# eichenberger/stereo-svo-slam

Measured on AMD Instinct MI355X. Metric: tracked_frames_per_sec, higher is better.
Workload: dtype f32

## Files before the change

include/svo_hip.h:

```cpp
#ifndef SVO_HIP_H
#define SVO_HIP_H

#include <stddef.h>

#include "svo_types.h"

#ifdef __cplusplus
extern "C" {
#endif

enum {
    SVO_OK = 0,
    SVO_ERR_INVALID = -1,
    SVO_ERR_HIP = -2,
    SVO_ERR_NO_DEVICE = -3,
    SVO_ERR_CAPACITY = -4
};

typedef struct svo_handle svo_handle;

const char *svo_last_error(void);
int svo_version(void);

int svo_handle_create(int device, int max_keypoints, svo_handle **out);
// ... 138 lines not shown
enum { SVO_KERNEL_SIA_GN = 0,
       SVO_KERNEL_REPROJ_GN = 1 };
typedef struct svo_launch_shape {
    int32_t kernel;
    int32_t waves;
    int32_t mode;
    int32_t cap;
    int64_t launches;
} svo_launch_shape;
int svo_ctx_get_launch_shapes(svo_ctx *ctx, svo_launch_shape *out, int max, int *n);
int svo_pick_launch_shapes(const svo_camera_settings *cam, int width, int height, int batch, int n_bound,
                           int rec_cap, int exact, svo_launch_shape out[2]);
int svo_pick_sia_lds_bytes(const svo_camera_settings *cam, int width, int height, int batch, int n_bound,
                           int rec_cap, int exact, int64_t *lds_bytes);

int svo_pinv6_check(svo_handle *h, const float *H_dev, int n, float *out_dev, int32_t *sweeps_dev, int impl);
int svo_solve6_check(svo_handle *h, const float *H_dev, const float *b_dev, int n, float *out_dev,
                     int32_t *sweeps_dev, int impl);

#ifdef __cplusplus
}
#endif
#endif
```

stereo-svo-slam_amd/csrc/klt.hip:

```cpp
#include "svo_kernels.hpp"
#include "klt_bounds.hpp"
#include <cstring>
#include <utility>

namespace svo {

constexpr int KLT_MAX_WIN = 35;
static_assert(KLT_MAX_WIN + 1 <= 36, "largest kernel shape");
#ifndef SVO_KLT_MARGIN
#define SVO_KLT_MARGIN 4
#endif
constexpr int KLT_MARGIN = SVO_KLT_MARGIN;
template <int CW>
struct KltGeom {
    static constexpr int DW = CW;
    static constexpr int RS = 44;
    static constexpr int RROWS = CW + 2;
    static constexpr int TJROWS = DW + 2 * KLT_MARGIN + 2;
    static constexpr int TJS = (DW + 2 * KLT_MARGIN + 6) & ~3;
    static constexpr int J2S = (TJS / 2) | 1;
    static constexpr int J2COPY = ((TJROWS * J2S + 31) / 32) * 32 + 16;
    static constexpr int SD = (DW + 1) * DW;
    static constexpr int SJ2 = J2COPY + TJROWS * J2S;
    static constexpr int SI = (RROWS * RS + 3) / 4;
// ... 113 lines not shown

#define M24(a, b) __mul24((a), (b))

__device__ inline int cv_round(float v) { return (int)rintf(v); }
__device__ inline int cv_floor(float v) { return (int)floorf(v); }

struct LkWeights { v2s top, bot; };

enum { KLT_OUTSIDE = 0, KLT_FLAT = 1, KLT_TRACK = 2 };
struct KltTmplHeader { int state; float A11, A12, A22; double cI1, cI2; };
template <int NPAIR>
struct KltTmpl {
    static constexpr int TQ = (3 * NPAIR + 3) / 4;
    static constexpr int BYTES = TQ * 64 * 16 + 64;
};
__device__ inline LkWeights lk_weights(float fa, float fb) {
    const int W_BITS = 14;
    const int iw00 = cv_round((1.f - fa) * (1.f - fb) * (1 << W_BITS));
    const int iw01 = cv_round(fa * (1.f - fb) * (1 << W_BITS));
    const int iw10 = cv_round((1.f - fa) * fb * (1 << W_BITS));
    const int iw11 = (1 << W_BITS) - iw00 - iw01 - iw10;
    return LkWeights{as_v2s(pack16(iw00, iw01)), as_v2s(pack16(iw10, iw11))};
}

template <int LS, int MAXROWS>
__device__ inline void stage_tile(uint8_t* tile, const ImgView& im, int x0, int y0, int nq, int rows) {
    const int tid = threadIdx.x;
    const bool fast = klt_rect_in_image(x0, y0, 4 * nq, rows, im.w, im.h) &&
                      (((reinterpret_cast<uintptr_t>(im.data) | (uintptr_t)im.stride) & 3) == 0);
    if (fast) {
// ... 87 lines not shown
                    const int gy = reflect101(y0 + min(r + u, rows - 1), im.h);
                    v[u] = im.g()[M24(gy, im.stride) + gx];
                }
#pragma unroll
                for (int u = 0; u < 8; u++)
                    if (r + u < rows) {
                        const uint16_t pv = (uint16_t)((int)v[u] << 7);
                        t16[(r + u) * 2 * KLT_J2S + tcol] = pv;
                        if (tcol > 0) t16[2 * KLT_J2COPY + (r + u) * 2 * KLT_J2S + tcol - 1] = pv;
                    }
            }
        }
    }
}

template <int CW>
__device__ __forceinline__ void klt_track_body(const KltArgs* __restrict__ args) {
    constexpr int NG = KLT_THREADS / CW;
    constexpr int ROWS = CW;
    constexpr int RPT = (((ROWS + NG - 1) / NG) + 1) & ~1;
    constexpr int NPAIR = RPT / 2;
    const KltArgs& a = args[blockIdx.y];
    const int n = *G(a.n_ptr);
    const int kp = blockIdx.x;
    if (kp >= n) return;
    const int tid = threadIdx.x;
#ifdef SVO_KLT_PHASES
    unsigned long long t_phase_ = __builtin_amdgcn_s_memtime();
    KLT_COUNT(8, 1);
#endif
    const int win = a.win;
    const int RW = win + 3, DW = win + 1, TJ = DW + 2 * KLT_MARGIN;
    const int lr = tid / CW, lc = tid - lr * CW;
    const bool row_on = lr < NG;
    const int y0 = row_on ? lr * RPT : 0;

    using GEO = KltGeom<CW>;
    constexpr int KLT_DW = GEO::DW, KLT_RS = GEO::RS, KLT_RROWS = GEO::RROWS, KLT_J2S = GEO::J2S, KLT_J2COPY = GEO::J2COPY;
    __shared__ __attribute__((aligned(16))) int s_mem[GEO::LDS_DWORDS];
    int* const s_d = s_mem;
    uint8_t* const s_I = reinterpret_cast<uint8_t*>(s_mem + GEO::SD);
    uint32_t* const s_J2 = reinterpret_cast<uint32_t*>(s_mem);
    __shared__ double s_part[KLT_WAVES][8];

    const int kfid = __builtin_amdgcn_readfirstlane(a.kf_id ? G(a.kf_id)[kp] : 0);
    SVO_GP(const KfDev) kfp = G(a.kfs) + kfid;

    svo_kp2d ref;
    float nx, ny;
    if (a.proj_pose) {
        const CamD camd = make_camd(a.cam.fx, a.cam.fy, a.cam.cx, a.cam.cy, a.cam);
        svo_kp2d q;
        if (a.proj_mats) {
            const PoseMats pm = *G(a.proj_mats);
            q = project_point(pm.Rd, pm.t, camd, G(a.kps3d)[kp]);
        } else {
            float pose[6];
            for (int i = 0; i < 6; i++) pose[i] = G(a.proj_pose)[i];
            PoseMats pm;
            pose_mats(pose, pm);
            q = project_point(pm.Rd, pm.t, camd, G(a.kps3d)[kp]);
        }
        nx = q.x; ny = q.y;
        ref = G(kfp->kps2d)[G(a.kp_index)[kp]];
        if (tid == 0) {
            G(a.proj_out)[kp] = q;
            if (a.ref_out) G(a.ref_out)[kp] = ref;
        }
    } else {
        ref = G(a.prev_pts)[kp];
        const svo_kp2d q = G(a.cur_pts)[kp];
        nx = q.x; ny = q.y;
    }

    const uint8_t* tmpl_base = (a.proj_pose && kfp->tmpl_win == a.win) ? (const uint8_t*)kfp->tmpl : nullptr;
    const int tmpl_cap = kfp->tmpl_cap;
    SVO_GP(uint8_t) tmpl_valid = G(kfp->tmpl_valid);
    const int kpi = a.proj_pose ? __builtin_amdgcn_readfirstlane(G(a.kp_index)[kp]) : 0;
    const int maxLevel = min(kfp->n_lk, a.n_cur) - 1;
    const float halfWin = (win - 1) * 0.5f;
    const int W_BITS = 14;
    const float FLT_SCALE = 1.f / (1 << 20);
    double epsilon = 0.01;
    epsilon *= epsilon;
    int status = 1;
    float err = 0;
    const bool col_on = row_on && lc < win;

    KLT_PHASE(0);
    for (int level = maxLevel; level >= 0; level--) {
        const ImgView J = a.cur[level];
        const float lscale = (float)(1. / (1 << level));
        float prevx = ref.x * lscale, prevy = ref.y * lscale;
        if (level == maxLevel) { nx = nx * lscale; ny = ny * lscale; }
        else { nx = nx * 2.f; ny = ny * 2.f; }
        float nextx = nx, nexty = ny;

        int tIw[NPAIR], tIx[NPAIR], tIy[NPAIR];
        float A11 = 0, A12 = 0, A22 = 0;
        double cI1 = 0, cI2 = 0;
        int lstate = KLT_TRACK;
        LkWeights wt;
        SVO_GP(uint4) rec = nullptr;
        SVO_GP(uint8_t) vflag = nullptr;
        if (tmpl_base && kpi < tmpl_cap) {
            rec = (SVO_GP(uint4))(tmpl_base + ((size_t)kpi * SVO_LK_LEVELS + level) * KltTmpl<NPAIR>::BYTES);
            vflag = tmpl_valid + kpi * SVO_LK_LEVELS + level;
        }
        KLT_PHASE(5);
        const int TW = (TJ + 3 + 3) & ~3;
        int tx0 = 0, ty0 = 0;
        bool have_tile = false, tile_regs = false;
        KltTileRegs<GEO> pre;
        uint4 hq0 = make_uint4(0, 0, 0, 0), hq1 = hq0;
        uint4 tq[KltTmpl<NPAIR>::TQ];
        int flag = 0;
        if (vflag) {
            flag = *vflag;
            SVO_GP(const uint4) hd = rec + KltTmpl<NPAIR>::TQ * 64;
            hq0 = hd[0]; hq1 = hd[1];
#pragma unroll
            for (int q = 0; q < KltTmpl<NPAIR>::TQ; q++) tq[q] = rec[q * 64 + tid];
            const bool look = klt_corner_in_range(nextx - halfWin, nexty - halfWin, win, J.w, J.h);
            const int px = look ? cv_floor(nextx - halfWin) : 0, py = look ? cv_floor(nexty - halfWin) : 0;
            const int qx0 = (px - KLT_MARGIN) & ~3, qy0 = py - KLT_MARGIN;
            if (look && tile_in_image(J, qx0, qy0, TW >> 2, TJ)) {
                tile_j2_load<GEO>(pre, J, qx0, qy0, TW >> 2, TJ);
                tx0 = qx0; ty0 = qy0; tile_regs = true;
            }
        }
        KLT_PHASE_WAIT(6);
        const bool hit = flag != 0;
        if (hit) {
            static_assert(sizeof(KltTmplHeader) == 32, "two 16-byte loads");
            lstate = (int)hq0.x; A11 = __uint_as_float(hq0.y); A12 = __uint_as_float(hq0.z); A22 = __uint_as_float(hq0.w);
            cI1 = __builtin_bit_cast(double, ((unsigned long long)hq1.y << 32) | hq1.x);
            cI2 = __builtin_bit_cast(double, ((unsigned long long)hq1.w << 32) | hq1.z);
            if (lstate == KLT_TRACK) {
                const uint32_t* f = reinterpret_cast<const uint32_t*>(tq);
#pragma unroll
                for (int k = 0; k < NPAIR; k++) { tIw[k] = (int)f[k]; tIx[k] = (int)f[NPAIR + k]; tIy[k] = (int)f[2 * NPAIR + k]; }
            }
        } else {
        tile_regs = false;
        int lc_b = lc, y0_b = y0;
        asm volatile("" : "+v"(lc_b), "+v"(y0_b));
        const ImgView I = kfp->lk[level];
        prevx -= halfWin; prevy -= halfWin;
        if (!klt_corner_in_range(prevx, prevy, win, I.w, I.h)) {
            lstate = KLT_OUTSIDE;
        } else {
        const int iprevx = cv_floor(prevx), iprevy = cv_floor(prevy);
        wt = lk_weights(prevx - iprevx, prevy - iprevy);

        __syncthreads();
        const int ix0 = (iprevx - 1) & ~3;
        const int ox = iprevx - 1 - ix0;
        stage_tile<KLT_RS, KLT_RROWS>(s_I, I, ix0, iprevy - 1, (ox + RW + 3) >> 2, RW);
// ... 178 lines not shown
                break;
            }
            prevDx = dx; prevDy = dy;
        }
        KLT_PHASE(3);

        if (status && level == 0) {
            const float npx = nx - halfWin, npy = ny - halfWin;
            if (!klt_corner_in_range(npx, npy, win, J.w, J.h)) {
                status = 0;
                continue;
            }
            const int inx = cv_floor(npx), iny = cv_floor(npy);
            if (!have_tile || inx < tx0 || iny < ty0 || inx + DW > tx0 + TW || iny + DW > ty0 + TJ)
                load_tile(inx, iny);
            wt = lk_weights(npx - inx, npy - iny);
            int e = 0;
            if (col_on) {
                int jr[RPT + 1];
                load_pairs(inx - tx0, iny - ty0, jr);
#pragma unroll
                for (int k = 0; k < NPAIR; k++) {
                    const v2s diff = row_pair(jr, wt, k) - as_v2s(tIw[k]);
                    if (y0 + 2 * k < win) e += abs((int)diff.x);
                    if (y0 + 2 * k + 1 < win) e += abs((int)diff.y);
                }
            }
            double sE[1];
            {
                const int pe[1] = {e};
// ... 4 lines not shown
        }
    }

    KLT_PHASE(4);
    if (tid == 0) {
        G(a.cur_pts)[kp] = svo_kp2d{nx, ny};
        G(a.status)[kp] = (uint8_t)status;
        G(a.err)[kp] = status ? err : INFINITY;
    }
}

template <int CW>
__global__ void klt_track_kernel(const KltArgs* __restrict__ args);
template <>
__global__ __launch_bounds__(KLT_THREADS) __attribute__((amdgpu_waves_per_eu(4, 4))) void klt_track_kernel<32>(const KltArgs* __restrict__ args) {
    klt_track_body<32>(args);
}
template <>
__global__ __launch_bounds__(KLT_THREADS) __attribute__((amdgpu_waves_per_eu(2, 2))) void klt_track_kernel<36>(const KltArgs* __restrict__ args) {
    klt_track_body<36>(args);
}

#ifdef SVO_KLT_PHASES
}
extern "C" int svo_debug_klt_phases(unsigned long long* out16) {
    static unsigned long long host[1024][16];
    if (hipMemcpyFromSymbol(host, HIP_SYMBOL(svo::g_klt_phases), sizeof(host)) != hipSuccess) return -1;
    for (int i = 0; i < 16; i++) {
        out16[i] = 0;
        for (int s = 0; s < 1024; s++) out16[i] += host[s][i];
    }
    memset(host, 0, sizeof(host));
    return hipMemcpyToSymbol(HIP_SYMBOL(svo::g_klt_phases), host, sizeof(host)) == hipSuccess ? 0 : -1;
}
namespace svo {
#endif

size_t klt_template_bytes(int win) {
    return win + 1 <= 32 ? KltTmpl<8>::BYTES : KltTmpl<18>::BYTES;
}

void launch_klt(const KltArgs* d_args, int batch, int max_n, int win, hipStream_t stream) {
    if (max_n <= 0) return;
    if (win + 1 <= 32)
        hipLaunchKernelGGL(klt_track_kernel<32>, dim3(max_n, batch), dim3(KLT_THREADS), 0, stream, d_args);
    else
        hipLaunchKernelGGL(klt_track_kernel<36>, dim3(max_n, batch), dim3(KLT_THREADS), 0, stream, d_args);
}

}
```

stereo-svo-slam_amd/csrc/svo_device.hpp:

```cpp
#pragma once

#include <hip/hip_runtime.h>
#include <float.h>
#include <stdint.h>

#include "../../include/svo_types.h"
#include "../../include/svo_libm.h"

namespace svo {

#if defined(__HIP_DEVICE_COMPILE__)
#define SVO_GP(T) __attribute__((address_space(1))) T*
#else
#define SVO_GP(T) T*
#endif
template <class T>
__device__ __forceinline__ SVO_GP(T) G(T* p) { return (SVO_GP(T))p; }

struct ImgView {
    const uint8_t* data;
    int w, h, stride;
    __device__ __forceinline__ SVO_GP(const uint8_t) g() const { return (SVO_GP(const uint8_t))data; }
    __device__ __forceinline__ SVO_GP(uint8_t) gw() const { return (SVO_GP(uint8_t))data; }
};

__host__ __device__ inline ImgView make_view(const svo_image& im) {
    return ImgView{im.data, im.width, im.height, im.stride};
}

#define SVO_LDS(T) __attribute__((address_space(3))) T
template <bool LDS, typename T>
__device__ inline T mem_ld(const T* p, int i) {
// ... 755 lines not shown
```

stereo-svo-slam_amd/csrc/svo_group.hip:

```cpp
#include <hip/hip_runtime.h>

#include <algorithm>
#include <chrono>
#include <cmath>
#include <cstddef>
#include <cstdio>
#include <cstdlib>
#include <cstring>
#include <memory>
#include <new>
#include <vector>

#include "svo_group.hpp"
#include "svo_host.hpp"
#include "svo_tracker.hpp"

using namespace svo;

namespace {

struct PoseFilter {
    static constexpr int N = 12;
    float statePre[N], statePost[N];
    float A[N * N], Hm[N * N], Q[N * N], R[N * N];
// ... 114 lines not shown
};

struct Seq {
    KpsDev kps[2];
    int cur = 0;
    int* d_n = nullptr;
    svo_kp2d* tracked = nullptr;
    float* klt_err = nullptr;
    uint8_t* klt_status = nullptr;
    float* disparity = nullptr;
    float* sia_rec = nullptr;
    float* sia_kpws = nullptr;
    PoseMats* sia_mats = nullptr;
    uint8_t* tmpl_base = nullptr;
    uint8_t* tmpl_valid = nullptr;
    KfDev* d_kfs = nullptr;
    std::vector<KfHost> kfs;
    int kfs_retired = 0;
    DetCell* det = nullptr; int* n_det = nullptr;
    DetCell* sel = nullptr; int* sel_level = nullptr; int* sel_cell = nullptr; int* occupied = nullptr;
    uint32_t* color_lcg = nullptr;
    std::vector<std::unique_ptr<ImageSet>> sets;
    std::vector<ImageSet*> free_sets;
    ImageSet* cur_set = nullptr;
    ImageSet* prev_set = nullptr;
    PoseFilter kf;
    int frame_id = -1;
    int run = 0;
    double ts = 0;
    float pose[6] = {0, 0, 0, 0, 0, 0};
// ... 59 lines not shown
    PinnedPtr<RemapImg> remap_img_host;
    bool timing = false;
    bool failed = false;
    int exact_pinv = 1;
    Event ev[10];
    SetLayout set_layout;
    std::vector<uint8_t*> kf_slabs;
    int kf_slab_count = 0;
    size_t device_bytes = 0;
    std::vector<FinishedRun> finished;
    std::vector<uint8_t*> set_slabs;
    int tmpl_kf = 0, tmpl_cap = 0;
    size_t tmpl_block_bytes = 0, tmpl_valid_bytes = 0;
    svo_totals totals;
    std::vector<svo_launch_shape> launch_shapes;
    bool retire_kf_images = true;
    int image_sets = 0;
    double host_ms[8] = {0, 0, 0, 0, 0, 0, 0, 0};
    long host_steps = 0;
};

void GroupDelete::operator()(svo_group* c) const {
    (void)hipSetDevice(c->device);
    if (c->stream) (void)hipStreamSynchronize(c->stream.get());
    if (std::getenv("SVO_HOST_TIMING") && c->host_steps > 0) {
        static const char* names[7] = {"args", "launch", "pose_filter", "wait_frame", "kf_enqueue", "wait_kf", "bookkeeping"};
        std::fprintf(stderr, "[svo host ms/step over %ld steps]", c->host_steps);
        for (int i = 0; i < 7; i++) std::fprintf(stderr, " %s=%.3f", names[i], c->host_ms[i] / c->host_steps);
        std::fprintf(stderr, "\n");
    }
// ... 244 lines not shown
    c->d_inside = reinterpret_cast<int*>(db + res_bytes + n_bytes);
    return SVO_OK;
}

int alloc_sequence(svo_group* c, Seq& q, int s) {
    q.d_n = c->d_n_all + 2 * s;
    int rc = alloc_kps(c, q.kps[0], q.d_n);
    if (!rc) rc = alloc_kps(c, q.kps[1], q.d_n + 1);
    auto alloc = [&](auto** p, size_t count) { if (!rc) rc = dev_alloc(c, p, count); };
    const size_t cap = c->cap, cells = c->max_cells;
    alloc(&q.tracked, cap); alloc(&q.klt_err, cap); alloc(&q.klt_status, cap); alloc(&q.disparity, cap);
    alloc(&q.sia_rec, sia_rec_ws_floats(c->cam, c->rec_cap)); alloc(&q.sia_kpws, (size_t)9 * c->rec_cap);
    alloc(&q.sia_mats, 1); alloc(&q.d_kfs, c->max_kf);
    alloc(&q.det, SVO_MAX_PYRAMID_LEVELS * cells); alloc(&q.n_det, SVO_MAX_PYRAMID_LEVELS);
    alloc(&q.sel, cells); alloc(&q.sel_level, cells); alloc(&q.sel_cell, cells); alloc(&q.occupied, c->merge_cells);
    alloc(&q.color_lcg, 1);
    if (rc) return rc;
    q.kf.init();
    std::memset(&q.stats, 0, sizeof(q.stats));
    for (int i = 0; i < 4; i++)
        if ((rc = new_image_set(c, q))) return rc;
    return SVO_OK;
}

int alloc_template_cache(svo_group* c) {
    const int B = c->B;
    const int cells = (c->width / c->cam.grid_width) * (c->height / c->cam.grid_height);
    c->tmpl_cap = std::min(c->cap, cells + 64);
    c->tmpl_block_bytes = align_up((size_t)c->tmpl_cap * SVO_LK_LEVELS * klt_template_bytes(c->cam.window_size_opt_flow), 256);
    int K = c->tmpl_block_bytes <= ((size_t)8 << 20) ? 8 : 4;
    if (const char* e = std::getenv("SVO_KLT_CACHE_KF")) K = std::max(0, std::min(std::atoi(e), 64));
// ... 17 lines not shown
}

int grp_create(const svo_camera_settings* cam, int width, int height, int n_sequences, int device, Group* out) {
    int rc = check_settings(cam, width, height, n_sequences);
    if (rc) return rc;
    int count = 0;
    if (hipGetDeviceCount(&count) != hipSuccess || count <= 0)
        return svo_set_error(SVO_ERR_NO_DEVICE, "no HIP device visible: libsvo_hip has no CPU fallback");
    if (device < 0 || device >= count) return svo_set_error(SVO_ERR_INVALID, "device %d out of range", device);
    HIP_TRY(hipSetDevice(device));
    Group g(new (std::nothrow) svo_group());
    svo_group* c = g.get();
    if (!c) return svo_set_error(SVO_ERR_INVALID, "out of host memory");
    c->device = device; c->B = n_sequences; c->width = width; c->height = height; c->cam = *cam;
    std::memset(&c->totals, 0, sizeof(c->totals));
    HIP_TRY(make_stream(c->stream));
    size_group(c);
    if ((rc = alloc_blocks(c))) return rc;
    for (Event& e : c->ev) HIP_TRY(make_event(e));
    c->seqs.resize(n_sequences);
    if ((rc = grow_set_slabs(c, 4 * n_sequences))) return rc;
    for (int s = 0; s < n_sequences; s++)
        if ((rc = alloc_sequence(c, c->seqs[s], s))) return rc;
    if ((rc = grow_kf_slabs(c, std::max(2 * n_sequences, 32)))) return rc;
    if ((rc = alloc_template_cache(c))) return rc;
    HIP_TRY(pinned_malloc(c->remap_img_host, sizeof(RemapImg) * 2 * (size_t)n_sequences));
    c->remap_img.h = c->remap_img_host.get();
    if ((rc = dev_alloc(c, &c->remap_img.d, 2 * (size_t)n_sequences))) return rc;
    HIP_TRY(hipDeviceSynchronize());
    *out = std::move(g);
// ... 168 lines not shown
    const KpsDev& k = q.kps[q.cur];
    sa.left = q.cur_set->left[0]; sa.right = q.cur_set->right;
    sa.n_ptr = k.n; sa.kps2d = k.kps2d; sa.disparity = q.disparity;
    sa.win = c->cam.window_size_depth_calculator; sa.search_x = c->cam.search_x;
    sa.search_y = c->cam.search_y; sa.clamp_half = clamp_half;
    sa.first = 0; sa.first_ptr = first_ptr;
}

void pack_tracking_args(svo_group* c, const Step& st) {
    ArgBlocks& a = c->args;
    for (int slot = 0; slot < (int)st.trk.size(); slot++) {
        const int s = st.trk[slot];
        Seq& q = c->seqs[s];
        FrameResult* dr = c->d_res + s;
        for (int i = 0; i < 6; i++) a.guess.h[s][i] = q.pending ? q.kf.statePost[i] : q.kf.statePre[i];
        pack_compact(c, q, slot, 0).min_kf = &dr->min_kf;
        const KpsDev& k = q.kps[q.cur];
        SiaArgs& sa = clear(a.sia.h[slot]);
        for (int l = 0; l < c->cam.max_pyramid_levels; l++) {
            sa.prev[l] = q.prev_set->left[l];
            sa.cur[l] = q.cur_set->left[l];
        }
        sa.cam = c->cam; sa.n_ptr = k.n; sa.kps2d = k.kps2d; sa.kps3d = k.kps3d; sa.flags = k.flags;
        sa.pose_guess = a.guess.d[s]; sa.pose_out = dr->pose_sia; sa.cost_out = &dr->sia_cost;
        sa.trace = dr->sia_trace; sa.kp_ws = q.sia_kpws;
        sa.rec_ws = q.sia_rec; sa.rec_cap = c->rec_cap;
        sa.mats_out = q.sia_mats;
        sa.dbg_H = nullptr; sa.dbg_level = -1; sa.cap = c->cap; sa.exact_pinv = c->exact_pinv;
        KltArgs& ka = clear(a.klt.h[slot]);
        ka.kfs = q.d_kfs; ka.kf_id = k.kf_id; ka.n_cur = c->n_lk;
        for (int l = 0; l < c->n_lk; l++) ka.cur[l] = q.cur_set->lk[l];
        ka.n_ptr = k.n; ka.prev_pts = nullptr; ka.cur_pts = q.tracked; ka.status = q.klt_status;
        ka.err = q.klt_err; ka.win = c->cam.window_size_opt_flow;
        ka.proj_pose = dr->pose_sia; ka.proj_mats = q.sia_mats; ka.kps3d = k.kps3d; ka.proj_out = k.kps2d;
        ka.kp_index = k.kp_index; ka.ref_out = nullptr; ka.cam = c->cam;
        ReprojArgs& ra = clear(a.reproj.h[slot]);
        ra.cam = c->cam; ra.n_ptr = k.n; ra.kps2d = k.kps2d; ra.kps3d = k.kps3d; ra.flags = k.flags;
        ra.tracked = q.tracked; ra.err = q.klt_err; ra.pose_in = dr->pose_sia;
        ra.pose_out = dr->pose_refined; ra.cost_out = &dr->reproj_cost; ra.trace = &dr->reproj_trace;
        ra.exact_pinv = c->exact_pinv;
        ra.zero_out = c->d_inside + s;
        pack_ssd(c, q, slot, 1, nullptr);
        FilterArgs& fa = clear(a.filter.h[slot]);
        fa.cam = c->cam; fa.n_ptr = k.n; fa.frame_pose = dr->pose_refined;
        fa.kps2d = k.kps2d; fa.kps3d = k.kps3d; fa.flags = k.flags;
        fa.outlier_count = k.outl; fa.inlier_count = k.inl; fa.kf_inv_depth = k.kfx;
        fa.kf_variance = k.kfP; fa.disparity = q.disparity;
        fa.kfs = q.d_kfs; fa.kf_id = k.kf_id; fa.kp_index = k.kp_index;
        fa.do_outlier_check = 1; fa.do_update = 1; fa.do_flags = 1; fa.do_reproject = 1;
        fa.width = c->width; fa.height = c->height; fa.inside_count = c->d_inside + s;
// ... 32 lines not shown
    }
    launch_compact(a.compact.d, T, c->cap, st);
    HIP_TRY(hipGetLastError());
    HIP_TRY(mark(c, 2));
    int grid_n = 1;
    for (int seq : s.trk) grid_n = std::max(grid_n, c->seqs[seq].n_host);
    grid_n = std::min(grid_n, c->cap);
    const LaunchStatus sia_launch =
        launch_sia(a.sia.d, T, c->cam, c->width, c->height, grid_n, c->rec_cap, c->exact_pinv, st);
    HIP_TRY(sia_launch.err);
    if (!sia_launch.shape.fits)
        return svo_set_error(SVO_ERR_CAPACITY, "sparse alignment: %d keypoints exceed the workspaces", grid_n);
    count_launch(c, SVO_KERNEL_SIA_GN, sia_launch.shape);
    HIP_TRY(hipGetLastError());
    HIP_TRY(mark(c, 3));
    launch_klt(a.klt.d, T, grid_n, c->cam.window_size_opt_flow, st);
    HIP_TRY(hipGetLastError());
    HIP_TRY(mark(c, 4));
    const LaunchStatus reproj_launch = launch_reproj(a.reproj.d, T, grid_n, st);
    HIP_TRY(reproj_launch.err);
    if (!reproj_launch.shape.fits)
        return svo_set_error(SVO_ERR_CAPACITY, "reprojection GN: %d keypoints do not fit LDS", grid_n);
    count_launch(c, SVO_KERNEL_REPROJ_GN, reproj_launch.shape);
    HIP_TRY(hipGetLastError());
    HIP_TRY(mark(c, 5));
    launch_ssd(a.ssd.d, T, grid_n, c->cam.window_size_depth_calculator, c->cam.search_y, st);
    HIP_TRY(hipGetLastError());
    HIP_TRY(mark(c, 6));
    launch_filter(a.filter.d, T, grid_n, st);
    HIP_TRY(hipGetLastError());
    HIP_TRY(mark(c, 7));
    HIP_TRY(hipMemcpyAsync(c->h_inside, c->d_inside, sizeof(int) * c->B, hipMemcpyDeviceToHost, st));
// ... 43 lines not shown
    for (int seq = 0; seq < c->B; seq++) {
        if (!s.need[seq]) continue;
        const int rc = pack_keyframe_args(c, m++, seq, s.start[seq] != 0);
        if (rc) return rc;
    }
    if (m == 0) return SVO_OK;
    HIP_TRY(hipMemcpyAsync(a.dev, a.host.get(), a.bytes, hipMemcpyHostToDevice, st));
    launch_compact(a.compact.d, m, c->cap, st);
    HIP_TRY(hipGetLastError());
    if (c->det_levels > 0) {
        launch_detect(a.detect.d, m, c->max_cells, c->det_levels, c->cam.grid_width, c->cam.grid_height, st);
        HIP_TRY(hipGetLastError());
    }
    launch_select_merge(a.merge.d, m, c->max_cells, st);
    HIP_TRY(hipGetLastError());
    launch_ssd(a.ssd.d, m, c->cap, c->cam.window_size_depth_calculator, c->cam.search_y, st);
    HIP_TRY(hipGetLastError());
    launch_kf_init(a.kf_init.d, m, st);
    HIP_TRY(hipGetLastError());
    return SVO_OK;
}

int decide_keyframes(svo_group* c, Step& s) {
    const int max_keypoints = (c->width / c->cam.grid_width) * (c->height / c->cam.grid_height);
    bool any = false;
    for (int seq : s.act) {
        s.need[seq] = s.start[seq] || (double)c->h_inside[seq] < 0.66 * max_keypoints ? 1 : 0;
        any = any || s.need[seq];
    }
    return any ? enqueue_keyframes(c, s) : SVO_OK;
}
// ... 249 lines not shown
                               float filtered[6]) {
    svo_group* c; int s;
    if (const int rc = ctx_seq(ctx, seq, &c, &s)) return rc;
    flush_pending(c);
    c->seqs[s].kf.update(pose, speed, pose_var, speed_var, dt, filtered);
    return SVO_OK;
}

extern "C" int svo_get_frame_stats(svo_ctx* ctx, int seq, svo_frame_stats* out) {
    svo_group* c; int s;
    if (const int rc = ctx_seq(ctx, seq, &c, &s)) return rc;
    if (out) *out = c->seqs[s].stats;
    return SVO_OK;
}

extern "C" int svo_get_finished_runs(svo_ctx* ctx, int seq, int* n) {
    svo_group* c; int s;
    if (const int rc = ctx_seq(ctx, seq, &c, &s)) return rc;
    if (n) *n = (int)std::count_if(c->finished.begin(), c->finished.end(), [s](const FinishedRun& f) { return f.info.seq == s; });
    return SVO_OK;
}

extern "C" int svo_get_finished_run(svo_ctx* ctx, int seq, int i, svo_run_info* info, svo_pose* trajectory,
                                    int cap, int* n_poses) {
    svo_group* c; int s;
    if (const int rc = ctx_seq(ctx, seq, &c, &s)) return rc;
    int k = 0;
    for (const FinishedRun& f : c->finished) {
        if (f.info.seq != s || k++ != i) continue;
        if (info) { *info = f.info; info->seq = seq; }
// ... 8 lines not shown
```

stereo-svo-slam_amd/csrc/svo_kernels.hpp:

```cpp
#pragma once

#include <hip/hip_runtime.h>
#include <mutex>

#include "svo_device.hpp"

namespace svo {

constexpr int SVO_MAX_DEVICES = 64;
struct LdsLimit {
    std::once_flag once[SVO_MAX_DEVICES];
    hipError_t err[SVO_MAX_DEVICES];
};
inline hipError_t raise_lds_limit(LdsLimit& st, const void* kernel, int bytes) {
    int dev = 0;
    hipError_t e = hipGetDevice(&dev);
    if (e != hipSuccess) return e;
    if (dev < 0 || dev >= SVO_MAX_DEVICES) return hipErrorInvalidDevice;
    std::call_once(st.once[dev], [&st, dev, kernel, bytes] {
        st.err[dev] = hipFuncSetAttribute(kernel, hipFuncAttributeMaxDynamicSharedMemorySize, bytes);
    });
    return st.err[dev];
}

// ... 86 lines not shown
    ImgView cur[SVO_LK_LEVELS];
    int n_cur;
    const int* n_ptr;
    const svo_kp2d* prev_pts;
    svo_kp2d* cur_pts;
    uint8_t* status;
    float* err;
    int win;
    const float* proj_pose;
    const PoseMats* proj_mats;
    const svo_kp3d* kps3d;
    svo_kp2d* proj_out;
    const int* kp_index;
    svo_kp2d* ref_out;
    svo_camera_settings cam;
};
void launch_klt(const KltArgs* d_args, int batch, int max_n, int win, hipStream_t stream);
size_t klt_template_bytes(int win);

struct ReprojArgs {
    svo_camera_settings cam;
    const int* n_ptr;
    svo_kp2d* kps2d;
    const svo_kp3d* kps3d;
    uint32_t* flags;
    const svo_kp2d* tracked;
    const float* err;
    const float* pose_in;
    float* pose_out;
    float* cost_out;
    svo_gn_trace* trace;
    int exact_pinv;
// ... 46 lines not shown
```

stereo-svo-slam_amd/stereo_svo_slam_amd/hip_lib.py:

```python
import ctypes as C
import os

import numpy as np
import torch

_HERE = os.path.dirname(os.path.abspath(__file__))
CSRC = os.path.normpath(os.path.join(_HERE, "..", "csrc"))
LIB_PATH = os.environ.get("SVO_HIP_LIB", os.path.join(CSRC, "libsvo_hip.so"))
_LIB = None

SYMBOLS = (
    "svo_last_error", "svo_version", "svo_handle_create", "svo_handle_destroy",
    "svo_handle_set_stream", "svo_handle_synchronize", "svo_build_pyramid",
    "svo_build_lk_pyramid", "svo_sparse_align", "svo_klt_track", "svo_reproj_gn",
    "svo_ssd_disparity", "svo_depth_filter_update",
    "svo_ctx_create", "svo_ctx_destroy", "svo_new_images", "svo_submit_images", "svo_wait",
    "svo_ctx_get_groups", "svo_new_image", "svo_get_pose",
    "svo_get_frame_keypoints", "svo_get_keyframe_count", "svo_get_keyframe",
    "svo_get_trajectory", "svo_update_pose", "svo_get_frame_stats", "svo_ctx_enable_timing",
    "svo_get_totals", "svo_handle_set_exact_pinv", "svo_ctx_set_exact_pinv",
    "svo_handle_set_fast_solver", "svo_ctx_set_fast_solver",
    "svo_device_malloc", "svo_device_free", "svo_copy_to_device", "svo_copy_to_host",
    "svo_copy_image_to_device", "svo_project_keypoints",
    "svo_ctx_get_launch_shapes", "svo_pick_launch_shapes", "svo_pick_sia_lds_bytes", "svo_pinv6_check",
    "svo_solve6_check", "svo_remap_linear", "svo_ctx_set_rectification",
    "svo_detect_keypoints", "svo_detect_shape",
    "svo_ctx_restart_sequences", "svo_get_finished_runs", "svo_get_finished_run",
    "svo_drop_finished_runs", "svo_ctx_get_memory",
)


class SvoError(RuntimeError):
    pass


class CameraSettings(C.Structure):
    _fields_ = [(n, C.c_float) for n in
                ("baseline", "fx", "fy", "cx", "cy", "k1", "k2", "k3", "p1", "p2")] + \
               [(n, C.c_int32) for n in
                ("grid_height", "grid_width", "search_x", "search_y",
                 "window_size_pose_estimator", "window_size_opt_flow",
                 "window_size_depth_calculator", "max_pyramid_levels",
                 "min_pyramid_level_pose_estimation")]
# ... 224 lines not shown
```

stereo-svo-slam_amd/stereo_svo_slam_amd/stereo_slam.py:

```python
import ctypes as C

import numpy as np
import torch

from . import hip_lib
from .hip_lib import CameraSettings, SvoError, _check, lib

KP_INFO_DTYPE = np.dtype([
    ("score", "<f4"), ("level", "<i4"), ("type", "<i4"), ("keyframe_id", "<i4"),
    ("keypoint_index", "<i4"), ("color", "u1", (3,)), ("ignore_during_refinement", "u1"),
    ("ignore_completely", "u1"), ("ignore_temporary", "u1"), ("_pad", "u1", (2,)),
    ("outlier_count", "<i4"), ("inlier_count", "<i4"), ("kf_inv_depth", "<f4"),
    ("kf_variance", "<f4")], align=False)
assert KP_INFO_DTYPE.itemsize == 44


class GnTrace(C.Structure):
    _fields_ = [("level", C.c_int32), ("n_gradient", C.c_int32), ("n_cost", C.c_int32),
                ("n_accepted", C.c_int32), ("exit_small", C.c_int32),
                ("initial_cost", C.c_float), ("final_cost", C.c_float), ("pose", C.c_float * 6)]


class FrameStats(C.Structure):
    _fields_ = [("frame_id", C.c_int32), ("is_keyframe", C.c_int32), ("n_keypoints", C.c_int32),
# ... 208 lines not shown
        _check(lib().svo_ctx_get_groups(self._ctx, C.byref(n)))
        return n.value

    def totals(self):
        t = Totals()
        _check(lib().svo_get_totals(self._ctx, C.byref(t)))
        return t

    def launch_shapes(self):
        n = C.c_int(0)
        _check(lib().svo_ctx_get_launch_shapes(self._ctx, None, 0, C.byref(n)))
        out = (LaunchShape * max(n.value, 1))()
        _check(lib().svo_ctx_get_launch_shapes(self._ctx, out, n.value, C.byref(n)))
        return {_shape_key(e): e.launches for e in out[:n.value]}

    def pose(self, seq=0):
        p = np.zeros(6, np.float32)
        _check(lib().svo_get_pose(self._ctx, seq, p.ctypes.data_as(C.c_void_p)))
        return p

    def stats(self, seq=0):
        st = FrameStats()
        _check(lib().svo_get_frame_stats(self._ctx, seq, C.byref(st)))
        return st

    def get_frame(self, seq=0):
        n = C.c_int(0)
        _check(lib().svo_get_frame_keypoints(self._ctx, seq, None, None, None, 0, C.byref(n)))
        k2 = np.zeros((n.value, 2), np.float32)
        k3 = np.zeros((n.value, 3), np.float32)
# ... 66 lines not shown
```

Baseline: 260,100.

## Split KLT tracking into hot cached-template kernel and cold fallback kernel

Splits KLT tracking into two kernels. The hot kernel handles keypoints whose keyframe templates are all cached and valid. It reads headers and per-level images through scalar constant-address loads, preloads the template gradients, and never builds templates. Keypoints it cannot serve go onto a miss list through an atomic counter, and a second cold kernel processes only that list along the original full path. This is meant to shrink register and branch cost on the common path, at the price of an extra launch, a counter-zeroing step and atomics. It also caps the SSD launch grid at max_cells.

```diff
diff --git a/include/svo_hip.h b/include/svo_hip.h
--- a/include/svo_hip.h
+++ b/include/svo_hip.h
@@ -176,6 +176,9 @@
 int svo_pick_sia_lds_bytes(const svo_camera_settings *cam, int width, int height, int batch, int n_bound,
                            int rec_cap, int exact, int64_t *lds_bytes);
 
+int svo_debug_klt_split(svo_ctx *ctx, int seq, int *hot, int *cold, svo_kp2d *tracked, uint8_t *status,
+                        float *err, int cap);
+
 int svo_pinv6_check(svo_handle *h, const float *H_dev, int n, float *out_dev, int32_t *sweeps_dev, int impl);
 int svo_solve6_check(svo_handle *h, const float *H_dev, const float *b_dev, int n, float *out_dev,
                      int32_t *sweeps_dev, int impl);
diff --git a/stereo-svo-slam_amd/csrc/klt.hip b/stereo-svo-slam_amd/csrc/klt.hip
--- a/stereo-svo-slam_amd/csrc/klt.hip
+++ b/stereo-svo-slam_amd/csrc/klt.hip
@@ -1,6 +1,7 @@
 #include "svo_kernels.hpp"
 #include "klt_bounds.hpp"
 #include <cstring>
+#include <type_traits>
 #include <utility>
 
 namespace svo {
@@ -151,6 +152,16 @@
     static constexpr int TQ = (3 * NPAIR + 3) / 4;
     static constexpr int BYTES = TQ * 64 * 16 + 64;
 };
+template <bool CONST>
+__device__ __forceinline__ int load_uniform(const int* p) {
+    if constexpr (CONST) return *(SVO_KP(const int))p;
+    else return __builtin_amdgcn_readfirstlane(*G(p));
+}
+typedef uint32_t u32x8 __attribute__((ext_vector_type(8)));
+__device__ inline KltTmplHeader load_header_uniform(const uint8_t* p) {
+    static_assert(sizeof(KltTmplHeader) == sizeof(u32x8), "one 32-byte load");
+    return __builtin_bit_cast(KltTmplHeader, *(SVO_KP(const u32x8))p);
+}
 __device__ inline LkWeights lk_weights(float fa, float fb) {
     const int W_BITS = 14;
     const int iw00 = cv_round((1.f - fa) * (1.f - fb) * (1 << W_BITS));
@@ -268,20 +279,37 @@
     }
 }
 
-template <int CW>
-__device__ __forceinline__ void klt_track_body(const KltArgs* __restrict__ args) {
+enum { KLT_FULL = 0, KLT_HOT = 1, KLT_COLD = 2 };
+enum { KLT_MISS_COUNT = 0, KLT_MISS_N = 1, KLT_MISS_LIST = 2 };
+#ifndef SVO_KLT_PREFETCH
+#define SVO_KLT_PREFETCH 0
+#endif
+#ifndef SVO_KLT_LATE_I
+#define SVO_KLT_LATE_I 0
+#endif
+template <class T>
+__device__ __forceinline__ T pick3(int l, const T& v0, const T& v1, const T& v2) { return l == 0 ? v0 : (l == 1 ? v1 : v2); }
+static_assert(SVO_LK_LEVELS == 3, "pick3");
+template <int CW, int MODE>
+__device__ __forceinline__ void klt_track_body(const KltArgs* __restrict__ args, int force_cold) {
     constexpr int NG = KLT_THREADS / CW;
     constexpr int ROWS = CW;
     constexpr int RPT = (((ROWS + NG - 1) / NG) + 1) & ~1;
     constexpr int NPAIR = RPT / 2;
     const KltArgs& a = args[blockIdx.y];
     const int n = *G(a.n_ptr);
-    const int kp = blockIdx.x;
-    if (kp >= n) return;
     const int tid = threadIdx.x;
+    int kp = blockIdx.x;
+    if constexpr (MODE == KLT_COLD) {
+        if (kp >= G(a.miss)[KLT_MISS_COUNT]) return;
+        kp = __builtin_amdgcn_readfirstlane(G(a.miss)[KLT_MISS_LIST + kp]);
+    } else {
+        if (MODE == KLT_HOT && kp == 0 && tid == 0) G(a.miss)[KLT_MISS_N] = n;
+        if (kp >= n) return;
+    }
 #ifdef SVO_KLT_PHASES
     unsigned long long t_phase_ = __builtin_amdgcn_s_memtime();
-    KLT_COUNT(8, 1);
+    if (MODE != KLT_HOT) KLT_COUNT(8, 1);
 #endif
     const int win = a.win;
     const int RW = win + 3, DW = win + 1, TJ = DW + 2 * KLT_MARGIN;
@@ -297,12 +325,49 @@
     uint32_t* const s_J2 = reinterpret_cast<uint32_t*>(s_mem);
     __shared__ double s_part[KLT_WAVES][8];
 
-    const int kfid = __builtin_amdgcn_readfirstlane(a.kf_id ? G(a.kf_id)[kp] : 0);
-    SVO_GP(const KfDev) kfp = G(a.kfs) + kfid;
+    const int kfid = a.kf_id ? load_uniform<MODE == KLT_HOT>(a.kf_id + kp) : 0;
+    using KfPtr = std::conditional_t<MODE == KLT_HOT, SVO_KP(const KfDev), SVO_GP(const KfDev)>;
+    KfPtr kfp = (KfPtr)a.kfs + kfid;
+
+    const bool proj = MODE != KLT_FULL || a.proj_pose != nullptr;
+    const uint8_t* tmpl_base = (proj && kfp->tmpl_win == a.win) ? (const uint8_t*)kfp->tmpl : nullptr;
+    const int tmpl_cap = kfp->tmpl_cap;
+    SVO_GP(uint8_t) tmpl_valid = G(kfp->tmpl_valid);
+    const int kpi = proj ? load_uniform<MODE == KLT_HOT>(a.kp_index + kp) : 0;
+    const int maxLevel = min(kfp->n_lk, a.n_cur) - 1;
+
+    constexpr int TQ_I = NPAIR / 4, TQ_D = 2 * NPAIR / 4;
+    static_assert(MODE != KLT_HOT || NPAIR % 4 == 0, "I, Ix and Iy of a lane are whole 16-byte pieces");
+    [[maybe_unused]] KltTmplHeader hd0{}, hd1{}, hd2{};
+    [[maybe_unused]] ImgView cv0{}, cv1{}, cv2{};
+    [[maybe_unused]] SVO_GP(const uint4) rec_kp = nullptr;
+    [[maybe_unused]] uint4 nq[TQ_D];
+    [[maybe_unused]] bool take = false;
+    [[maybe_unused]] uint32_t fw0 = 0, fw1 = 0;
+    if constexpr (MODE == KLT_HOT) {
+        take = !force_cold && tmpl_base && kpi < tmpl_cap && maxLevel >= 0;
+        if (take) {
+            const int o = kpi * SVO_LK_LEVELS;
+            const int last = (tmpl_cap * SVO_LK_LEVELS - 1) >> 2;
+            SVO_KP(const uint32_t) fw = (SVO_KP(const uint32_t))kfp->tmpl_valid;
+            fw0 = fw[o >> 2]; fw1 = fw[min((o >> 2) + 1, last)];
+            const uint8_t* r0 = tmpl_base + (size_t)kpi * SVO_LK_LEVELS * KltTmpl<NPAIR>::BYTES;
+            constexpr int HDR = KltTmpl<NPAIR>::TQ * 64 * 16;
+            hd0 = load_header_uniform(r0 + HDR);
+            hd1 = load_header_uniform(r0 + KltTmpl<NPAIR>::BYTES + HDR);
+            hd2 = load_header_uniform(r0 + 2 * KltTmpl<NPAIR>::BYTES + HDR);
+            SVO_KP(const ImgView) cur = (SVO_KP(const ImgView))a.cur;
+            cv0 = cur[0]; cv1 = cur[1]; cv2 = cur[2];
+            rec_kp = (SVO_GP(const uint4))r0;
+            SVO_GP(const uint4) r = rec_kp + (size_t)maxLevel * (KltTmpl<NPAIR>::BYTES / 16);
+#pragma unroll
+            for (int q = 0; q < TQ_D; q++) nq[q] = r[(TQ_I + q) * 64 + tid];
+        }
+    }
 
     svo_kp2d ref;
     float nx, ny;
-    if (a.proj_pose) {
+    if (proj) {
         const CamD camd = make_camd(a.cam.fx, a.cam.fy, a.cam.cx, a.cam.cy, a.cam);
         svo_kp2d q;
         if (a.proj_mats) {
@@ -316,7 +381,7 @@
             q = project_point(pm.Rd, pm.t, camd, G(a.kps3d)[kp]);
         }
         nx = q.x; ny = q.y;
-        ref = G(kfp->kps2d)[G(a.kp_index)[kp]];
+        ref = G(kfp->kps2d)[kpi];
         if (tid == 0) {
             G(a.proj_out)[kp] = q;
             if (a.ref_out) G(a.ref_out)[kp] = ref;
@@ -327,11 +392,21 @@
         nx = q.x; ny = q.y;
     }
 
-    const uint8_t* tmpl_base = (a.proj_pose && kfp->tmpl_win == a.win) ? (const uint8_t*)kfp->tmpl : nullptr;
-    const int tmpl_cap = kfp->tmpl_cap;
-    SVO_GP(uint8_t) tmpl_valid = G(kfp->tmpl_valid);
-    const int kpi = a.proj_pose ? __builtin_amdgcn_readfirstlane(G(a.kp_index)[kp]) : 0;
-    const int maxLevel = min(kfp->n_lk, a.n_cur) - 1;
+    if constexpr (MODE == KLT_HOT) {
+        if (take) {
+            const uint32_t f3 = (uint32_t)((((unsigned long long)fw1 << 32) | fw0) >> ((kpi * SVO_LK_LEVELS & 3) * 8));
+            for (int l = 0; l <= maxLevel; l++) take = take && ((f3 >> (8 * l)) & 0xffu) != 0;
+        }
+        if (!take) {
+            if (tid == 0) {
+                const int e = __hip_atomic_fetch_add(G(a.miss) + KLT_MISS_COUNT, 1, __ATOMIC_RELAXED, __HIP_MEMORY_SCOPE_AGENT);
+                G(a.miss)[KLT_MISS_LIST + e] = kp;
+            }
+            return;
+        }
+        KLT_COUNT(8, 1);
+    }
+
     const float halfWin = (win - 1) * 0.5f;
     const int W_BITS = 14;
     const float FLT_SCALE = 1.f / (1 << 20);
@@ -341,9 +416,16 @@
     float err = 0;
     const bool col_on = row_on && lc < win;
 
+    [[maybe_unused]] int nq_level = maxLevel;
     KLT_PHASE(0);
     for (int level = maxLevel; level >= 0; level--) {
-        const ImgView J = a.cur[level];
+        ImgView J;
+        if constexpr (MODE == KLT_HOT) {
+            J.data = pick3(level, cv0.data, cv1.data, cv2.data); J.w = pick3(level, cv0.w, cv1.w, cv2.w);
+            J.h = pick3(level, cv0.h, cv1.h, cv2.h); J.stride = pick3(level, cv0.stride, cv1.stride, cv2.stride);
+        } else {
+            J = a.cur[level];
+        }
         const float lscale = (float)(1. / (1 << level));
         float prevx = ref.x * lscale, prevy = ref.y * lscale;
         if (level == maxLevel) { nx = nx * lscale; ny = ny * lscale; }
@@ -357,7 +439,7 @@
         LkWeights wt;
         SVO_GP(uint4) rec = nullptr;
         SVO_GP(uint8_t) vflag = nullptr;
-        if (tmpl_base && kpi < tmpl_cap) {
+        if (MODE != KLT_HOT && tmpl_base && kpi < tmpl_cap) {
             rec = (SVO_GP(uint4))(tmpl_base + ((size_t)kpi * SVO_LK_LEVELS + level) * KltTmpl<NPAIR>::BYTES);
             vflag = tmpl_valid + kpi * SVO_LK_LEVELS + level;
         }
@@ -369,7 +451,51 @@
         uint4 hq0 = make_uint4(0, 0, 0, 0), hq1 = hq0;
         uint4 tq[KltTmpl<NPAIR>::TQ];
         int flag = 0;
-        if (vflag) {
+        if constexpr (MODE == KLT_HOT) {
+            lstate = pick3(level, hd0.state, hd1.state, hd2.state);
+            A11 = pick3(level, hd0.A11, hd1.A11, hd2.A11); A12 = pick3(level, hd0.A12, hd1.A12, hd2.A12);
+            A22 = pick3(level, hd0.A22, hd1.A22, hd2.A22);
+            cI1 = pick3(level, hd0.cI1, hd1.cI1, hd2.cI1); cI2 = pick3(level, hd0.cI2, hd1.cI2, hd2.cI2);
+            if (lstate == KLT_TRACK) {
+#if SVO_KLT_PREFETCH
+                if (level != nq_level) {
+                    SVO_GP(const uint4) r = rec_kp + (size_t)level * (KltTmpl<NPAIR>::BYTES / 16);
+#pragma unroll
+                    for (int q = 0; q < TQ_D; q++) nq[q] = r[(TQ_I + q) * 64 + tid];
+                }
+#pragma unroll
+                for (int q = 0; q < TQ_D; q++) tq[TQ_I + q] = nq[q];
+                nq_level = level - 1;
+                if (nq_level >= 0) {
+                    SVO_GP(const uint4) r = rec_kp + (size_t)nq_level * (KltTmpl<NPAIR>::BYTES / 16);
+#pragma unroll
+                    for (int q = 0; q < TQ_D; q++) nq[q] = r[(TQ_I + q) * 64 + tid];
+                }
+#else
+                if (level == maxLevel) {
+#pragma unroll
+                    for (int q = 0; q < TQ_D; q++) tq[TQ_I + q] = nq[q];
+                } else {
+                    SVO_GP(const uint4) r = rec_kp + (size_t)level * (KltTmpl<NPAIR>::BYTES / 16);
+#pragma unroll
+                    for (int q = 0; q < TQ_D; q++) tq[TQ_I + q] = r[(TQ_I + q) * 64 + tid];
+                }
+#endif
+#if !SVO_KLT_LATE_I
+                if (level == 0) {
+#pragma unroll
+                    for (int q = 0; q < TQ_I; q++) tq[q] = rec_kp[q * 64 + tid];
+                }
+#endif
+                const bool look = klt_corner_in_range(nextx - halfWin, nexty - halfWin, win, J.w, J.h);
+                const int px = look ? cv_floor(nextx - halfWin) : 0, py = look ? cv_floor(nexty - halfWin) : 0;
+                const int qx0 = (px - KLT_MARGIN) & ~3, qy0 = py - KLT_MARGIN;
+                if (look && tile_in_image(J, qx0, qy0, TW >> 2, TJ)) {
+                    tile_j2_load<GEO>(pre, J, qx0, qy0, TW >> 2, TJ);
+                    tx0 = qx0; ty0 = qy0; tile_regs = true;
+                }
+            }
+        } else if (vflag) {
             flag = *vflag;
             SVO_GP(const uint4) hd = rec + KltTmpl<NPAIR>::TQ * 64;
             hq0 = hd[0]; hq1 = hd[1];
@@ -385,7 +511,19 @@
         }
         KLT_PHASE_WAIT(6);
         const bool hit = flag != 0;
-        if (hit) {
+        if constexpr (MODE == KLT_HOT) {
+            if (lstate == KLT_TRACK) {
+                const uint32_t* f = reinterpret_cast<const uint32_t*>(tq);
+#pragma unroll
+                for (int k = 0; k < NPAIR; k++) { tIx[k] = (int)f[NPAIR + k]; tIy[k] = (int)f[2 * NPAIR + k]; }
+#if !SVO_KLT_LATE_I
+                if (level == 0) {
+#pragma unroll
+                    for (int k = 0; k < NPAIR; k++) tIw[k] = (int)f[k];
+                }
+#endif
+            }
+        } else if (hit) {
             static_assert(sizeof(KltTmplHeader) == 32, "two 16-byte loads");
             lstate = (int)hq0.x; A11 = __uint_as_float(hq0.y); A12 = __uint_as_float(hq0.z); A22 = __uint_as_float(hq0.w);
             cI1 = __builtin_bit_cast(double, ((unsigned long long)hq1.y << 32) | hq1.x);
@@ -395,7 +533,7 @@
 #pragma unroll
                 for (int k = 0; k < NPAIR; k++) { tIw[k] = (int)f[k]; tIx[k] = (int)f[NPAIR + k]; tIy[k] = (int)f[2 * NPAIR + k]; }
             }
-        } else {
+        } else if constexpr (MODE != KLT_HOT) {
         tile_regs = false;
         int lc_b = lc, y0_b = y0;
         asm volatile("" : "+v"(lc_b), "+v"(y0_b));
@@ -604,6 +742,16 @@
             const int inx = cv_floor(npx), iny = cv_floor(npy);
             if (!have_tile || inx < tx0 || iny < ty0 || inx + DW > tx0 + TW || iny + DW > ty0 + TJ)
                 load_tile(inx, iny);
+#if SVO_KLT_LATE_I
+            if constexpr (MODE == KLT_HOT) {
+                uint4 iq[TQ_I];
+#pragma unroll
+                for (int q = 0; q < TQ_I; q++) iq[q] = rec_kp[q * 64 + tid];
+                const uint32_t* f = reinterpret_cast<const uint32_t*>(iq);
+#pragma unroll
+                for (int k = 0; k < NPAIR; k++) tIw[k] = (int)f[k];
+            }
+#endif
             wt = lk_weights(npx - inx, npy - iny);
             int e = 0;
             if (col_on) {
@@ -638,11 +786,17 @@
 __global__ void klt_track_kernel(const KltArgs* __restrict__ args);
 template <>
 __global__ __launch_bounds__(KLT_THREADS) __attribute__((amdgpu_waves_per_eu(4, 4))) void klt_track_kernel<32>(const KltArgs* __restrict__ args) {
-    klt_track_body<32>(args);
+    klt_track_body<32, KLT_FULL>(args, 0);
+}
+__global__ __launch_bounds__(KLT_THREADS) __attribute__((amdgpu_waves_per_eu(4, 4))) void klt_hot_kernel(const KltArgs* __restrict__ args, int force_cold) {
+    klt_track_body<32, KLT_HOT>(args, force_cold);
+}
+__global__ __launch_bounds__(KLT_THREADS) __attribute__((amdgpu_waves_per_eu(4, 4))) void klt_cold_kernel(const KltArgs* __restrict__ args) {
+    klt_track_body<32, KLT_COLD>(args, 0);
 }
 template <>
 __global__ __launch_bounds__(KLT_THREADS) __attribute__((amdgpu_waves_per_eu(2, 2))) void klt_track_kernel<36>(const KltArgs* __restrict__ args) {
-    klt_track_body<36>(args);
+    klt_track_body<36, KLT_FULL>(args, 0);
 }
 
 #ifdef SVO_KLT_PHASES
@@ -672,4 +826,21 @@
         hipLaunchKernelGGL(klt_track_kernel<36>, dim3(max_n, batch), dim3(KLT_THREADS), 0, stream, d_args);
 }
 
-}
+hipError_t launch_klt_split(const KltArgs* d_args, int batch, int max_n, int win, bool force_cold, hipStream_t stream) {
+    if (max_n <= 0) return hipSuccess;
+#ifdef SVO_KLT_NOFOLD
+    const bool split = false;
+#else
+    const bool split = win + 1 <= 32;
+#endif
+    if (!split) {
+        launch_klt(d_args, batch, max_n, win, stream);
+        return hipGetLastError();
+    }
+    hipLaunchKernelGGL(klt_hot_kernel, dim3(max_n, batch), dim3(KLT_THREADS), 0, stream, d_args, force_cold ? 1 : 0);
+    if (const hipError_t e = hipGetLastError(); e != hipSuccess) return e;
+    hipLaunchKernelGGL(klt_cold_kernel, dim3(max_n, batch), dim3(KLT_THREADS), 0, stream, d_args);
+    return hipGetLastError();
+}
+
+}
diff --git a/stereo-svo-slam_amd/csrc/svo_device.hpp b/stereo-svo-slam_amd/csrc/svo_device.hpp
--- a/stereo-svo-slam_amd/csrc/svo_device.hpp
+++ b/stereo-svo-slam_amd/csrc/svo_device.hpp
@@ -16,6 +16,11 @@
 #endif
 template <class T>
 __device__ __forceinline__ SVO_GP(T) G(T* p) { return (SVO_GP(T))p; }
+#if defined(__HIP_DEVICE_COMPILE__)
+#define SVO_KP(T) __attribute__((address_space(4))) T*
+#else
+#define SVO_KP(T) T*
+#endif
 
 struct ImgView {
     const uint8_t* data;
diff --git a/stereo-svo-slam_amd/csrc/svo_group.hip b/stereo-svo-slam_amd/csrc/svo_group.hip
--- a/stereo-svo-slam_amd/csrc/svo_group.hip
+++ b/stereo-svo-slam_amd/csrc/svo_group.hip
@@ -152,6 +152,7 @@
     PoseMats* sia_mats = nullptr;
     uint8_t* tmpl_base = nullptr;
     uint8_t* tmpl_valid = nullptr;
+    int* klt_miss = nullptr;
     KfDev* d_kfs = nullptr;
     std::vector<KfHost> kfs;
     int kfs_retired = 0;
@@ -241,6 +242,7 @@
     size_t tmpl_block_bytes = 0, tmpl_valid_bytes = 0;
     svo_totals totals;
     std::vector<svo_launch_shape> launch_shapes;
+    bool klt_force_cold = false;
     bool retire_kf_images = true;
     int image_sets = 0;
     double host_ms[8] = {0, 0, 0, 0, 0, 0, 0, 0};
@@ -515,7 +517,7 @@
     alloc(&q.sia_mats, 1); alloc(&q.d_kfs, c->max_kf);
     alloc(&q.det, SVO_MAX_PYRAMID_LEVELS * cells); alloc(&q.n_det, SVO_MAX_PYRAMID_LEVELS);
     alloc(&q.sel, cells); alloc(&q.sel_level, cells); alloc(&q.sel_cell, cells); alloc(&q.occupied, c->merge_cells);
-    alloc(&q.color_lcg, 1);
+    alloc(&q.color_lcg, 1); alloc(&q.klt_miss, 2 + cap);
     if (rc) return rc;
     q.kf.init();
     std::memset(&q.stats, 0, sizeof(q.stats));
@@ -563,6 +565,7 @@
     if (!c) return svo_set_error(SVO_ERR_INVALID, "out of host memory");
     c->device = device; c->B = n_sequences; c->width = width; c->height = height; c->cam = *cam;
     std::memset(&c->totals, 0, sizeof(c->totals));
+    if (const char* e = std::getenv("SVO_KLT_FORCE_COLD")) c->klt_force_cold = std::atoi(e) != 0;
     HIP_TRY(make_stream(c->stream));
     size_group(c);
     if ((rc = alloc_blocks(c))) return rc;
@@ -761,7 +764,9 @@
         Seq& q = c->seqs[s];
         FrameResult* dr = c->d_res + s;
         for (int i = 0; i < 6; i++) a.guess.h[s][i] = q.pending ? q.kf.statePost[i] : q.kf.statePre[i];
-        pack_compact(c, q, slot, 0).min_kf = &dr->min_kf;
+        CompactArgs& ca = pack_compact(c, q, slot, 0);
+        ca.min_kf = &dr->min_kf;
+        ca.zero = q.klt_miss; ca.zero_count = 1;
         const KpsDev& k = q.kps[q.cur];
         SiaArgs& sa = clear(a.sia.h[slot]);
         for (int l = 0; l < c->cam.max_pyramid_levels; l++) {
@@ -780,7 +785,7 @@
         ka.n_ptr = k.n; ka.prev_pts = nullptr; ka.cur_pts = q.tracked; ka.status = q.klt_status;
         ka.err = q.klt_err; ka.win = c->cam.window_size_opt_flow;
         ka.proj_pose = dr->pose_sia; ka.proj_mats = q.sia_mats; ka.kps3d = k.kps3d; ka.proj_out = k.kps2d;
-        ka.kp_index = k.kp_index; ka.ref_out = nullptr; ka.cam = c->cam;
+        ka.kp_index = k.kp_index; ka.ref_out = nullptr; ka.cam = c->cam; ka.miss = q.klt_miss;
         ReprojArgs& ra = clear(a.reproj.h[slot]);
         ra.cam = c->cam; ra.n_ptr = k.n; ra.kps2d = k.kps2d; ra.kps3d = k.kps3d; ra.flags = k.flags;
         ra.tracked = q.tracked; ra.err = q.klt_err; ra.pose_in = dr->pose_sia;
@@ -843,8 +848,7 @@
     count_launch(c, SVO_KERNEL_SIA_GN, sia_launch.shape);
     HIP_TRY(hipGetLastError());
     HIP_TRY(mark(c, 3));
-    launch_klt(a.klt.d, T, grid_n, c->cam.window_size_opt_flow, st);
-    HIP_TRY(hipGetLastError());
+    HIP_TRY(launch_klt_split(a.klt.d, T, grid_n, c->cam.window_size_opt_flow, c->klt_force_cold, st));
     HIP_TRY(mark(c, 4));
     const LaunchStatus reproj_launch = launch_reproj(a.reproj.d, T, grid_n, st);
     HIP_TRY(reproj_launch.err);
@@ -918,7 +922,7 @@
     }
     launch_select_merge(a.merge.d, m, c->max_cells, st);
     HIP_TRY(hipGetLastError());
-    launch_ssd(a.ssd.d, m, c->cap, c->cam.window_size_depth_calculator, c->cam.search_y, st);
+    launch_ssd(a.ssd.d, m, std::min(c->cap, c->max_cells), c->cam.window_size_depth_calculator, c->cam.search_y, st);
     HIP_TRY(hipGetLastError());
     launch_kf_init(a.kf_init.d, m, st);
     HIP_TRY(hipGetLastError());
@@ -1198,6 +1202,22 @@
     return SVO_OK;
 }
 
+extern "C" int svo_debug_klt_split(svo_ctx* ctx, int seq, int* hot, int* cold, svo_kp2d* tracked, uint8_t* status,
+                                   float* err, int cap) {
+    svo_group* c; int s;
+    if (const int rc = ctx_seq(ctx, seq, &c, &s)) return rc;
+    const Seq& q = c->seqs[s];
+    int v[2] = {0, 0};
+    if (q.frame_id > 0) HIP_TRY(hipMemcpy(v, q.klt_miss, sizeof(v), hipMemcpyDeviceToHost));
+    if (hot) *hot = v[1] - v[0];
+    if (cold) *cold = v[0];
+    const size_t n = (size_t)std::max(0, std::min({cap, v[1], c->cap}));
+    if (n && tracked) HIP_TRY(hipMemcpy(tracked, q.tracked, n * sizeof(svo_kp2d), hipMemcpyDeviceToHost));
+    if (n && status) HIP_TRY(hipMemcpy(status, q.klt_status, n, hipMemcpyDeviceToHost));
+    if (n && err) HIP_TRY(hipMemcpy(err, q.klt_err, n * sizeof(float), hipMemcpyDeviceToHost));
+    return SVO_OK;
+}
+
 extern "C" int svo_get_finished_runs(svo_ctx* ctx, int seq, int* n) {
     svo_group* c; int s;
     if (const int rc = ctx_seq(ctx, seq, &c, &s)) return rc;
diff --git a/stereo-svo-slam_amd/csrc/svo_kernels.hpp b/stereo-svo-slam_amd/csrc/svo_kernels.hpp
--- a/stereo-svo-slam_amd/csrc/svo_kernels.hpp
+++ b/stereo-svo-slam_amd/csrc/svo_kernels.hpp
@@ -124,8 +124,10 @@
     const int* kp_index;
     svo_kp2d* ref_out;
     svo_camera_settings cam;
+    int* miss;
 };
 void launch_klt(const KltArgs* d_args, int batch, int max_n, int win, hipStream_t stream);
+hipError_t launch_klt_split(const KltArgs* d_args, int batch, int max_n, int win, bool force_cold, hipStream_t stream);
 size_t klt_template_bytes(int win);
 
 struct ReprojArgs {
diff --git a/stereo-svo-slam_amd/stereo_svo_slam_amd/hip_lib.py b/stereo-svo-slam_amd/stereo_svo_slam_amd/hip_lib.py
--- a/stereo-svo-slam_amd/stereo_svo_slam_amd/hip_lib.py
+++ b/stereo-svo-slam_amd/stereo_svo_slam_amd/hip_lib.py
@@ -26,7 +26,7 @@
     "svo_solve6_check", "svo_remap_linear", "svo_ctx_set_rectification",
     "svo_detect_keypoints", "svo_detect_shape",
     "svo_ctx_restart_sequences", "svo_get_finished_runs", "svo_get_finished_run",
-    "svo_drop_finished_runs", "svo_ctx_get_memory",
+    "svo_drop_finished_runs", "svo_ctx_get_memory", "svo_debug_klt_split",
 )
 
 
diff --git a/stereo-svo-slam_amd/stereo_svo_slam_amd/stereo_slam.py b/stereo-svo-slam_amd/stereo_svo_slam_amd/stereo_slam.py
--- a/stereo-svo-slam_amd/stereo_svo_slam_amd/stereo_slam.py
+++ b/stereo-svo-slam_amd/stereo_svo_slam_amd/stereo_slam.py
@@ -246,6 +246,16 @@
         _check(lib().svo_ctx_get_launch_shapes(self._ctx, out, n.value, C.byref(n)))
         return {_shape_key(e): e.launches for e in out[:n.value]}
 
+    def klt_split(self, seq=0):
+        hot, cold = C.c_int(0), C.c_int(0)
+        _check(lib().svo_debug_klt_split(self._ctx, seq, C.byref(hot), C.byref(cold), None, None, None, 0))
+        n = hot.value + cold.value
+        tracked, status, err = np.zeros((n, 2), np.float32), np.zeros(n, np.uint8), np.zeros(n, np.float32)
+        _check(lib().svo_debug_klt_split(self._ctx, seq, C.byref(hot), C.byref(cold),
+                                         tracked.ctypes.data_as(C.c_void_p), status.ctypes.data_as(C.c_void_p),
+                                         err.ctypes.data_as(C.c_void_p), n))
+        return hot.value, cold.value, tracked, status, err
+
     def pose(self, seq=0):
         p = np.zeros(6, np.float32)
         _check(lib().svo_get_pose(self._ctx, seq, p.ctypes.data_as(C.c_void_p)))
```

Result: no change. 258,500 (-0.6%).
